# cwozny/sdr_channelizer

Hardware: AMD Instinct MI355X
Metric: input MS/s (complex) channelized (higher is better)
Workload: dtype f32; 1 GPU; cfg2: M=64 channels, 12 taps/branch, D=64, int16 I/Q (12-bit), 2^30 samples per GPU per step, frame-major complex64 out; kernel=pfb_fast<M64,P12,D64,int16>, schedule=default (4: FIR/FFT wave pairs, 8x64-frame workgroups), samples_per_gpu=1073741824, prewarm_steps=20, parallelism=single GPU

## Files before the change

sdr_channelizer_amd/csrc/pfb_fast_core.hpp:

```cpp
#pragma once

#include "pfb_fast_cfg.hpp"

namespace pfb {

template <class K, bool CM = false, bool MS = false>
struct FastKernel : FastRows<K> {
  static constexpr int M = K::M, P = K::P, D = K::D, CPT = K::CPT, C = K::C, W = K::W, OS = K::OS, NT = K::NT;
  static constexpr int NW = W - 1 + C;

  template <int I, bool FULL = false, int MAGSEL = -1, int NTSEL = -1>
  PFB_DEV void pass(const KernelParams& p, float2* src, float2* dst, int tid, long long f0,
                    const v2f (&tw)[2][16]) {
    float2* const p_out = p.out;
    const long long p_frames = p.frames;
    const int nontemporal = NTSEL < 0 ? p.nontemporal : NTSEL;
    constexpr int R = K::R(I), S = K::S(I), KK = K::K(I), RS = K::RS(I);
    constexpr int IPF = M / R, ITEMS = C * IPF, ITERS = (ITEMS + NT - 1) / NT;
    constexpr bool LAST = (I == K::NP - 1);
    constexpr bool TW_REGS = (ITERS == 1) && !K::TW_TABLE;
    constexpr bool READ_BARRIER = !LAST && !K::PINGPONG && NT > 64;
    constexpr bool kMagStaged = MS && LAST;
#pragma unroll
    for (int it = 0; it < ITERS; ++it) {
      const int w = tid + it * NT;
      const bool active = (ITEMS % NT == 0) || (w < ITEMS);
      const int fc = w / IPF, item = w % IPF;
      const int kk = item / S, rest = item % S;
      v2f x[R];
      if (active) {
        const v2f* s2 = reinterpret_cast<const v2f*>(src) + fc * K::FS + item;
#pragma unroll
        for (int n = 0; n < R; ++n) x[n] = s2[n * RS];
      } else {
#pragma unroll
        for (int n = 0; n < R; ++n) x[n] = (v2f){0.f, 0.f};
      }
      if constexpr (READ_BARRIER) __syncthreads();
      Dft<R>::run(x);
      if constexpr (!LAST) {
        constexpr int S1 = K::S(I + 1), RS1 = K::RS(I + 1);
        if constexpr (TW_REGS) {
#pragma unroll
          for (int k = 1; k < R; ++k) x[k] = cmul_w(x[k], tw[I][k]);
        } else {
          const float4* t4 = reinterpret_cast<const float4*>(p.tw_lane + K::TW_OFF(I) + rest * K::TWR(I));
#pragma unroll
          for (int k2 = 0; k2 < K::TWR(I) / 2; ++k2) {
            const float4 t = t4[k2];
            if (k2 > 0) x[2 * k2] = cmul_w(x[2 * k2], (v2f){t.x, t.y});
            if (2 * k2 + 1 < R) x[2 * k2 + 1] = cmul_w(x[2 * k2 + 1], (v2f){t.z, t.w});
          }
        }
        const int n1 = rest / S1, rest2 = rest % S1;
        if (active) {
          v2f* d2 = reinterpret_cast<v2f*>(dst) + fc * K::FS + n1 * RS1 + kk * S1 + rest2;
#pragma unroll
          for (int k = 0; k < R; ++k) d2[k * KK * S1] = x[k];
        }
      } else {
        if constexpr (kMagStaged) {
          static_assert(!CM && NT == 64 && ITERS == 1 && K::NP == 2 && !K::PINGPONG && M % 4 == 0, "single-wave two-pass plans");
          {
            constexpr int SR = M + ((8 - M % 64) + 64) % 64;
            static_assert(C * SR * sizeof(float) <= K::BUF * sizeof(float2), "the staged magnitudes fit the chunk buffer");
            float* stage = reinterpret_cast<float*>(src);
            const int shift = (p.flags & PFB_FLAG_FFTSHIFT) ? (M / 2) : 0;
            team_sync<true>();
#pragma unroll
            for (int k = 0; k < R; ++k) {
              int col = kk + k * KK + shift;
              col = col >= M ? col - M : col;
              if (active) stage[fc * SR + col] = mag_out(x[k].x, x[k].y, p.flags);
            }
            team_sync<true>();
            constexpr int NV = C * M / 4;
#pragma unroll
            for (int j = 0; j < (NV + 63) / 64; ++j) {
              const int idx = tid + 64 * j, fr = idx / (M / 4), q = idx % (M / 4);
              if ((NV % 64 == 0 || idx < NV) && f0 + fr < p_frames) {
                const float4 v = *reinterpret_cast<const float4*>(stage + fr * SR + q * 4);
                *reinterpret_cast<float4*>(reinterpret_cast<float*>(p_out) + (f0 + fr) * M + q * 4) = v;
              }
            }
            return;
          }
        }
        const long long f = f0 + fc;
        if (active && (FULL || f < p_frames)) {
          const bool flip_odd = (OS == 2) && (p.flags & PFB_FLAG_DEROTATE) && ((p.frame0 + f) & 1);
          const v2f sg0 = splat((flip_odd && (kk & 1)) ? -1.f : 1.f), sg1 = splat((flip_odd && ((kk + KK) & 1)) ? -1.f : 1.f);
          auto derot = [&](v2f v, int k) { return OS == 2 ? v * (((k * KK) & 1) ? sg1 : sg0) : v; };
          const int shift = (p.flags & PFB_FLAG_FFTSHIFT) ? (M / 2) : 0;
          auto col_of = [&](int ch) {
            const int c2 = ch + shift;
            return c2 >= M ? c2 - M : c2;
          };
          auto slot = [&](auto* rowp, int k) {
            if constexpr (K::POW2) {
              auto* lo = rowp + kk + shift;
              auto* hi = rowp + kk + (M / 2 - shift);
              return (k < R / 2) ? lo + k * KK : hi + (k - R / 2) * KK;
            } else {
              return rowp + col_of(kk + k * KK);
            }
          };
          if constexpr (CM || (!K::POW2 && K::NT == 64)) {
            const bool mag = MAGSEL < 0 ? (p.flags & PFB_FLAG_MAGNITUDE) != 0 : MAGSEL == 1;
            const long long esz = mag ? 4 : 8;
            const long long cs = CM ? p.out_ld : 1;
            int col = col_of(kk);
            char* ptr = reinterpret_cast<char*>(p_out) + ((long long)col * cs + (CM ? p.out_frame0 + f : f * M)) * esz;
            const long long step = (long long)KK * cs * esz, wrap = (long long)M * cs * esz;
#pragma unroll
            for (int k = 0; k < R; ++k) {
              v2f v = x[k];
              if (mag) {
                *reinterpret_cast<float*>(ptr) = mag_out(v.x, v.y, p.flags);
              } else {
                v = derot(v, k);
                store_c64(reinterpret_cast<float2*>(ptr), v, nontemporal);
              }
              asm volatile("" : "+v"(ptr) : : "memory");
              col += KK;
              ptr += step;
              if (col >= M) { col -= M; ptr -= wrap; }
            }
          } else if (MAGSEL == 1 || (MAGSEL < 0 && (p.flags & PFB_FLAG_MAGNITUDE))) {
            float* rowm = reinterpret_cast<float*>(p_out) + f0 * M + fc * M;
#pragma unroll
            for (int k = 0; k < R; ++k) *slot(rowm, k) = mag_out(x[k].x, x[k].y, p.flags);
          } else {
            float2* row = p_out + f0 * M + fc * M;
#pragma unroll
            for (int k = 0; k < R; ++k) {
              const v2f v = derot(x[k], k);
              store_c64(slot(row, k), v, nontemporal);
            }
          }
        }
      }
    }
  }

  PFB_DEV int tslot_frame(int col, int fc) {
    constexpr int IPF = M / K::R(K::NP - 1), NFC = IPF >= 16 ? 1 : 16 / IPF, Q = 16 / C;
    static_assert(16 % C == 0 && (IPF >= 16 || 16 % IPF == 0) && C % NFC == 0, "power-of-two chunk and lane groups");
    return fc ^ (NFC * ((col / Q) % (C / NFC)));
  }

  PFB_DEV void last_pass_transposed(const KernelParams& p, float2* slot, int tid, long long f0) {
    constexpr int I = K::NP - 1;
    constexpr int R = K::R(I), KK = K::K(I), RS = K::RS(I);
    constexpr int IPF = M / R, ITEMS = C * IPF, ITERS = (ITEMS + NT - 1) / NT;
    static_assert(NT == 64 && !K::PINGPONG && K::S(I) == 1 && M * C <= K::LDS_ELEMS, "wave-local, in place");
    v2f x[ITERS][R];
#pragma unroll
    for (int it = 0; it < ITERS; ++it) {
      const int w = tid + it * NT;
      const bool active = (ITEMS % NT == 0) || (w < ITEMS);
      const int fc = w / IPF, item = w % IPF;
      const v2f* s2 = reinterpret_cast<const v2f*>(slot) + fc * K::FS + item;
#pragma unroll
      for (int n = 0; n < R; ++n) x[it][n] = active ? s2[n * RS] : (v2f){0.f, 0.f};
    }
    team_sync<true>();
    const int shift = (p.flags & PFB_FLAG_FFTSHIFT) ? (M / 2) : 0;
    v2f* t2 = reinterpret_cast<v2f*>(slot);
#pragma unroll
    for (int it = 0; it < ITERS; ++it) {
      const int w = tid + it * NT;
      const bool active = (ITEMS % NT == 0) || (w < ITEMS);
      const int fc = w / IPF, kk = w % IPF;
      Dft<R>::run(x[it]);
      if (active) {
        const bool flip_odd = (OS == 2) && (p.flags & PFB_FLAG_DEROTATE) && ((p.frame0 + f0 + fc) & 1);
        const v2f sg0 = splat((flip_odd && (kk & 1)) ? -1.f : 1.f), sg1 = splat((flip_odd && ((kk + KK) & 1)) ? -1.f : 1.f);
        int col = kk + shift;
        if (col >= M) col -= M;
#pragma unroll
        for (int k = 0; k < R; ++k) {
          v2f v = x[it][k];
          if constexpr (OS == 2) v = v * (((k * KK) & 1) ? sg1 : sg0);
          t2[col * C + tslot_frame(col, fc)] = v;
          col += KK;
          if (col >= M) col -= M;
        }
      }
    }
  }

  struct Consts {
    v2f hp[(W + 1) / 2][CPT];
    v2f tw[2][16];
    int upos[OS][CPT];
    v2f conj_mul;
  };

  PFB_DEV float tap(const Consts& k, int j, int cc) { return (j & 1) ? k.hp[j >> 1][cc].y : k.hp[j >> 1][cc].x; }

  PFB_DEV void setup(const KernelParams& p, int tid, Consts& k) {
    const int c0 = tid * CPT;
#pragma unroll
    for (int cc = 0; cc < CPT; ++cc) {
      const int col = (K::LANES < NT && c0 >= D) ? 0 : c0 + cc;
      const float4* tl = reinterpret_cast<const float4*>(p.taps_lane + (size_t)col * K::WP);
#pragma unroll
      for (int q4 = 0; q4 < K::WP / 4; ++q4) {
        const float4 v = tl[q4];
        if (2 * q4 < (W + 1) / 2) k.hp[2 * q4][cc] = (v2f){v.x, v.y};
        if (2 * q4 + 1 < (W + 1) / 2) k.hp[2 * q4 + 1][cc] = (v2f){v.z, v.w};
      }
    }
    k.conj_mul = (v2f){1.f, (p.flags & PFB_FLAG_CONJUGATE_INPUT) ? -1.f : 1.f};
#pragma unroll
    for (int i = 0; i < K::NP - 1; ++i) {
      constexpr int dummy = 0; (void)dummy;
      const int R = K::R(i), S = K::S(i), IPF = M / R;
      if (C * IPF <= NT && !K::TW_TABLE) {
        const int rest = (tid % IPF) % S;
        const float4* t4 = reinterpret_cast<const float4*>(p.tw_lane + K::TW_OFF(i) + rest * K::TWR(i));
#pragma unroll
        for (int k2 = 0; k2 < 8; ++k2) {
          if (2 * k2 < R) {
            const float4 v = t4[k2];
            k.tw[i][2 * k2] = (v2f){v.x, v.y};
            k.tw[i][2 * k2 + 1] = (v2f){v.z, v.w};
          }
        }
      }
    }
#pragma unroll
    for (int ph = 0; ph < OS; ++ph)
#pragma unroll
      for (int cc = 0; cc < CPT; ++cc) {
        const int n = (D - 1 - (c0 + cc)) + D * ph;
        k.upos[ph][cc] = (n / K::S(0)) * K::RS(0) + (n % K::S(0));
      }
  }

  template <bool WAVE_LOCAL = false, bool TRANSPOSED = false, bool FULL = false, int MAGSEL = -1>
  PFB_DEV void fir_fft_store(const KernelParams& p, const Consts& k, const v2f (&x)[NW][CPT], float2* lds, int tid,
                             long long f0) {
    float2* buf0 = lds;
    float2* buf1 = K::PINGPONG ? lds + K::BUF : lds;
#pragma unroll
    for (int ph = 0; ph < OS; ++ph)
#pragma unroll
      for (int cc = 0; cc < CPT; ++cc) {
        v2f acc[C];
        int tok = 0;
#pragma unroll
        for (int q = 0; q < P; ++q) {
          const int j = ph + OS * q;
#pragma unroll
          for (int t = 0; t < C; ++t) {
            if (q == 0 && (j & 1)) fma_tap0_hi(acc[t], x[W - 1 + t - j][cc], k.hp[j >> 1][cc]);
            else if (q == 0) fma_tap0_lo(acc[t], x[W - 1 + t - j][cc], k.hp[j >> 1][cc]);
            else if (j & 1) fma_tap_hi(acc[t], x[W - 1 + t - j][cc], k.hp[j >> 1][cc], tok);
            else fma_tap_lo(acc[t], x[W - 1 + t - j][cc], k.hp[j >> 1][cc], tok);
          }
        }
        if (!(K::LANES < NT) || tid < K::LANES) {
#pragma unroll
          for (int t = 0; t < C; ++t)
            reinterpret_cast<v2f*>(buf0)[t * K::FS + k.upos[ph][cc]] = acc[t] * k.conj_mul;
        }
      }
    team_sync<WAVE_LOCAL>();
    pass<0>(p, buf0, buf1, tid, f0, k.tw);
    team_sync<WAVE_LOCAL>();
    if constexpr (TRANSPOSED) {
      static_assert(K::NP == 2 && WAVE_LOCAL, "single-wave two-pass plans");
      last_pass_transposed(p, buf1, tid, f0);
      return;
    } else if constexpr (K::NP == 2) {
      pass<1, FULL, MAGSEL>(p, buf1, nullptr, tid, f0, k.tw);
    } else {
      pass<1>(p, buf1, buf0, tid, f0, k.tw);
      team_sync<WAVE_LOCAL>();
      pass<2, FULL, MAGSEL>(p, buf0, nullptr, tid, f0, k.tw);
    }
    team_sync<WAVE_LOCAL>();
  }

  static constexpr bool kPairWrite = CPT == 2 && K::RS(0) == K::S(0) && K::S(0) % 2 == 0 && D % 2 == 0 && K::FS % 2 == 0 &&
                                     K::BUF % 2 == 0;
  PFB_DEV void fir_to_lds(const Consts& k, const v2f (&x)[NW][CPT], float2* buf, int tid) {
    if constexpr (kPairWrite) {
#pragma unroll
      for (int ph = 0; ph < OS; ++ph) {
        v2f acc[2][C];
#pragma unroll
        for (int cc = 0; cc < 2; ++cc) {
          int tok = 0;
#pragma unroll
          for (int q = 0; q < P; ++q) {
            const int j = ph + OS * q;
#pragma unroll
            for (int t = 0; t < C; ++t) {
              if (q == 0 && (j & 1)) fma_tap0_hi(acc[cc][t], x[W - 1 + t - j][cc], k.hp[j >> 1][cc]);
              else if (q == 0) fma_tap0_lo(acc[cc][t], x[W - 1 + t - j][cc], k.hp[j >> 1][cc]);
              else if (j & 1) fma_tap_hi(acc[cc][t], x[W - 1 + t - j][cc], k.hp[j >> 1][cc], tok);
              else fma_tap_lo(acc[cc][t], x[W - 1 + t - j][cc], k.hp[j >> 1][cc], tok);
            }
          }
        }
        if (!(K::LANES < NT) || tid < K::LANES) {
#pragma unroll
          for (int t = 0; t < C; ++t) {
            const v2f lo = acc[1][t] * k.conj_mul, hi = acc[0][t] * k.conj_mul;
            *reinterpret_cast<float4*>(buf + t * K::FS + k.upos[ph][1]) = make_float4(lo.x, lo.y, hi.x, hi.y);
          }
        }
      }
      return;
    }
#pragma unroll
    for (int ph = 0; ph < OS; ++ph)
#pragma unroll
      for (int cc = 0; cc < CPT; ++cc) {
        v2f acc[C];
        int tok = 0;
#pragma unroll
        for (int q = 0; q < P; ++q) {
          const int j = ph + OS * q;
#pragma unroll
          for (int t = 0; t < C; ++t) {
            if (q == 0 && (j & 1)) fma_tap0_hi(acc[t], x[W - 1 + t - j][cc], k.hp[j >> 1][cc]);
            else if (q == 0) fma_tap0_lo(acc[t], x[W - 1 + t - j][cc], k.hp[j >> 1][cc]);
            else if (j & 1) fma_tap_hi(acc[t], x[W - 1 + t - j][cc], k.hp[j >> 1][cc], tok);
            else fma_tap_lo(acc[t], x[W - 1 + t - j][cc], k.hp[j >> 1][cc], tok);
          }
        }
        if (!(K::LANES < NT) || tid < K::LANES) {
#pragma unroll
          for (int t = 0; t < C; ++t)
            reinterpret_cast<v2f*>(buf)[t * K::FS + k.upos[ph][cc]] = acc[t] * k.conj_mul;
        }
      }
  }

  template <bool FULL = false, int MAGSEL = -1, int NTSEL = -1>
  PFB_DEV void fft_from_lds(const KernelParams& p, const Consts& k, float2* buf, int tid, long long f0) {
    static_assert(K::NP == 2 && !K::PINGPONG, "two in-place passes");
    pass<0>(p, buf, buf, tid, f0, k.tw);
    team_sync<true>();
    pass<1, FULL, MAGSEL, NTSEL>(p, buf, nullptr, tid, f0, k.tw);
  }
};

}
```

sdr_channelizer_amd/csrc/pfb_fast_teams.hpp:

```cpp
#pragma once

#include "pfb_fast_core.hpp"

namespace pfb {

template <class K>
struct Teams : FastKernel<K> {
  using F = FastKernel<K>;
  using typename F::raw_t; using typename F::Consts;
  using F::cvt; using F::setup; using F::fir_to_lds;
  static constexpr int M = K::M, P = K::P, D = K::D, CPT = K::CPT, C = K::C, W = K::W, OS = K::OS, NT = K::NT, NW = F::NW;

  template <int I>
  PFB_DEV void pass_frame(const KernelParams& p, float2* fbuf, int lane, const v2f (&tw)[2][16]) {
    constexpr int R = K::R(I), S = K::S(I), KK = K::K(I), RS = K::RS(I);
    constexpr int IPF = M / R, ITERS = (IPF + 63) / 64;
    constexpr int S1 = K::S(I + 1), RS1 = K::RS(I + 1);
    static_assert(I < K::NP - 1, "the last pass (with the stores) belongs to the FIR team");
    constexpr bool TW_REGS = (ITERS == 1) && !K::TW_TABLE;
    v2f x[ITERS][R];
#pragma unroll
    for (int it = 0; it < ITERS; ++it) {
      const int item = lane + it * 64;
      const bool active = (IPF % 64 == 0) || (item < IPF);
      const v2f* s2 = reinterpret_cast<const v2f*>(fbuf) + (active ? item : 0);
#pragma unroll
      for (int n = 0; n < R; ++n) x[it][n] = s2[n * RS];
    }
#pragma unroll
    for (int it = 0; it < ITERS; ++it) {
      const int item = lane + it * 64;
      const bool active = (IPF % 64 == 0) || (item < IPF);
      const int kk = item / S, rest = item % S;
      Dft<R>::run(x[it]);
      if constexpr (TW_REGS) {
#pragma unroll
        for (int k = 1; k < R; ++k) x[it][k] = cmul_w(x[it][k], tw[I][k]);
      } else {
        const float4* t4 = reinterpret_cast<const float4*>(p.tw_lane + K::TW_OFF(I) + (active ? rest : 0) * K::TWR(I));
#pragma unroll
        for (int k2 = 0; k2 < K::TWR(I) / 2; ++k2) {
          const float4 t = t4[k2];
          if (k2 > 0) x[it][2 * k2] = cmul_w(x[it][2 * k2], (v2f){t.x, t.y});
          if (2 * k2 + 1 < R) x[it][2 * k2 + 1] = cmul_w(x[it][2 * k2 + 1], (v2f){t.z, t.w});
        }
      }
      if (active) {
        const int n1 = rest / S1, rest2 = rest % S1;
        v2f* d2 = reinterpret_cast<v2f*>(fbuf) + n1 * RS1 + kk * S1 + rest2;
#pragma unroll
        for (int k = 0; k < R; ++k) d2[k * KK * S1] = x[it][k];
      }
    }
  }

  template <bool INTERIOR, int MAGSEL = -1>
  PFB_DEV void fir_team(const KernelParams& p, const Consts& k, float2* bufs, long long f_begin, int nch) {
    const int tid = threadIdx.x;
    const int c0 = tid * CPT;
    auto last_pass = [&](float2* buf, int c) {
      int t2 = tid;
      asm volatile("" : "+v"(t2));
      F::template pass<K::NP - 1, INTERIOR, MAGSEL>(p, buf, nullptr, t2, f_begin + (long long)c * C, k.tw);
    };
    const raw_t* run_ptr = static_cast<const raw_t*>(p.in) + ((f_begin - (W - 1)) * D + p.base);
    v2f x[NW][CPT];
    raw_t raw[2][C][CPT];
#pragma unroll
    for (int i = 0; i < W - 1; ++i) {
      raw_t t[CPT];
      F::template load_row<INTERIOR>(p, run_ptr, f_begin - (W - 1) + i, i, c0, t);
#pragma unroll
      for (int cc = 0; cc < CPT; ++cc) x[i][cc] = cvt(t[cc]);
    }
#pragma unroll
    for (int u = 0; u < 2; ++u)
#pragma unroll
      for (int t = 0; t < C; ++t) F::template load_row<INTERIOR>(p, run_ptr, f_begin + u * C + t, W - 1 + u * C + t, c0, raw[u][t]);
    int b_fir = 0, b_last = 1;
    auto step = [&]<int U, bool LASTP>(int ci) {
      const long long f0 = f_begin + (long long)ci * C;
#pragma unroll
      for (int t = 0; t < C; ++t)
#pragma unroll
        for (int cc = 0; cc < CPT; ++cc) x[W - 1 + t][cc] = cvt(raw[U][t][cc]);
      if (ci + 2 < nch) {
        const long long rel = (long long)(ci + 2) * C + (W - 1);
#pragma unroll
        for (int t = 0; t < C; ++t) F::template load_row<INTERIOR>(p, run_ptr, f0 + 2 * C + t, rel + t, c0, raw[U][t]);
      }
      fir_to_lds(k, x, bufs + b_fir * K::BUF, tid);
#pragma unroll
      for (int i = 0; i < W - 1; ++i)
#pragma unroll
        for (int cc = 0; cc < CPT; ++cc) x[i][cc] = x[i + C][cc];
      if constexpr (LASTP) last_pass(bufs + b_last * K::BUF, ci - 2);
      __syncthreads();
      b_fir = (b_fir == 2) ? 0 : b_fir + 1;
      b_last = (b_last == 2) ? 0 : b_last + 1;
    };
    step.template operator()<0, false>(0);
    step.template operator()<1, false>(1);
    for (int ci2 = 2; ci2 < nch; ci2 += 2) {
      step.template operator()<0, true>(ci2);
      step.template operator()<1, true>(ci2 + 1);
    }
    if (nch >= 2) last_pass(bufs + b_last * K::BUF, nch - 2);
    __syncthreads();
    b_last = (b_last == 2) ? 0 : b_last + 1;
    last_pass(bufs + b_last * K::BUF, nch - 1);
  }

  template <int MAGSEL = -1>
  PFB_DEV void run_teams(const KernelParams& p, float2* bufs) {
    static_assert(K::NP == 3 && !K::PINGPONG && NT % 64 == 0, "three in-place passes");
    const int wave = threadIdx.x >> 6, lane = threadIdx.x & 63;
    const int nch = p.frames_per_block / C;
    Consts k;
    setup(p, wave < NT / 64 ? threadIdx.x : lane, k);
    long long run = blockIdx.x;
    run = xcd_remap_block(run, gridDim.x, p.xcd_remap);
    const long long f_begin = run * p.frames_per_block;
    if (f_begin >= p.frames) return;
    if (wave < NT / 64) {
      const bool interior = p.vec_ok && ((f_begin - (W - 1)) * D + p.base >= 0) && (f_begin + p.frames_per_block <= p.frames);
      if (interior) fir_team<true, MAGSEL>(p, k, bufs, f_begin, nch);
      else fir_team<false, MAGSEL>(p, k, bufs, f_begin, nch);
    } else {
      const int fr = wave - NT / 64;
      int b = 0;
#pragma unroll 1
      for (int s = 0; s <= nch; ++s) {
        if (s >= 1) {
          float2* fbuf = bufs + b * K::BUF + fr * K::FS;
          pass_frame<0>(p, fbuf, lane, k.tw);
          team_sync<true>();
          pass_frame<1>(p, fbuf, lane, k.tw);
          b = (b == 2) ? 0 : b + 1;
        }
        __syncthreads();
      }
    }
  }
};

template <class K>
constexpr bool kTeamsOk = !K::WAVE_FRAMES && K::NP == 3 && !K::PINGPONG && K::NT > 64 && (K::NT + 64 * K::C) <= 1024 &&
                          3 * sizeof(float2) * K::BUF <= 160 * 1024 && K::C % 2 == 0;

template <class K, bool MAG>
__global__ void __launch_bounds__(K::NT + 64 * K::C, K::MIN_WAVES) pfb_teams_kernel(const KernelParams p) {
  carry_history(p, SampleT<K::FMT>::kBytes, K::NT + 64 * K::C);
  __shared__ float2 bufs[3 * K::BUF];
  Teams<K>::template run_teams<MAG ? 1 : 0>(p, bufs);
}

template <class K>
KernelEntry teams_entry(const KernelParams& p) {
  static constexpr KernelTag mag = kernel_tag<>("teams", {.magsel = 1}), c64 = kernel_tag<>("teams", {.magsel = 0});
  return wants_magnitude(p) ? entry_for(&pfb_teams_kernel<K, true>, 6, mag.s, p, p.frames_per_block, K::NT + 64 * K::C)
                            : entry_for(&pfb_teams_kernel<K, false>, 6, c64.s, p, p.frames_per_block, K::NT + 64 * K::C);
}

}
```

Baseline: 484,800 MS/s.

## Peel interior FIR loop, use scalar-base prefetch loads, clamp last-pass lanes

The interior FIR team loop is restructured. The steady-state iterations now prefetch unconditionally, and the final two steps are peeled so they skip the prefetch. Prefetch loads use a new scalar-base-plus-vector-offset global load so address math stays in SGPRs, and sched_barriers plus an explicit waitcnt constrain instruction scheduling. The last FFT pass clamps out-of-range work items to a duplicate valid item instead of branching on activity. These changes aim to cut per-step address and branch overhead, but depend on hand-placed waitcnt encodings and scheduling fences that may reduce compiler freedom.

```diff
diff --git a/sdr_channelizer_amd/csrc/pfb_fast_core.hpp b/sdr_channelizer_amd/csrc/pfb_fast_core.hpp
--- a/sdr_channelizer_amd/csrc/pfb_fast_core.hpp
+++ b/sdr_channelizer_amd/csrc/pfb_fast_core.hpp
@@ -9,7 +9,7 @@
   static constexpr int M = K::M, P = K::P, D = K::D, CPT = K::CPT, C = K::C, W = K::W, OS = K::OS, NT = K::NT;
   static constexpr int NW = W - 1 + C;
 
-  template <int I, bool FULL = false, int MAGSEL = -1, int NTSEL = -1>
+  template <int I, bool FULL = false, int MAGSEL = -1, int NTSEL = -1, bool DUP = false>
   PFB_DEV void pass(const KernelParams& p, float2* src, float2* dst, int tid, long long f0,
                     const v2f (&tw)[2][16]) {
     float2* const p_out = p.out;
@@ -23,7 +23,7 @@
     constexpr bool kMagStaged = MS && LAST;
 #pragma unroll
     for (int it = 0; it < ITERS; ++it) {
-      const int w = tid + it * NT;
+      const int w = (DUP && tid + it * NT >= ITEMS) ? ITEMS - 1 : tid + it * NT;
       const bool active = (ITEMS % NT == 0) || (w < ITEMS);
       const int fc = w / IPF, item = w % IPF;
       const int kk = item / S, rest = item % S;
diff --git a/sdr_channelizer_amd/csrc/pfb_fast_teams.hpp b/sdr_channelizer_amd/csrc/pfb_fast_teams.hpp
--- a/sdr_channelizer_amd/csrc/pfb_fast_teams.hpp
+++ b/sdr_channelizer_amd/csrc/pfb_fast_teams.hpp
@@ -54,14 +54,28 @@
     }
   }
 
+  PFB_DEV void load_row_sbase(const raw_t* rowp, unsigned cbyte, raw_t (&raw)[CPT]) {
+    using RawVec = typename F::RawVec;
+    static_assert(sizeof(RawVec) % 4 == 0, "whole dwords per lane");
+    typedef unsigned dwords_t __attribute__((ext_vector_type(sizeof(RawVec) / 4)));
+    typedef const char __attribute__((address_space(1))) * gbytes_t;
+    uintptr_t base = reinterpret_cast<uintptr_t>(rowp);
+    asm volatile("" : "+s"(base), "+v"(cbyte));
+    const dwords_t v = *reinterpret_cast<const dwords_t __attribute__((address_space(1)))*>(
+        reinterpret_cast<gbytes_t>(base) + cbyte);
+    __builtin_memcpy(&raw[0], &v, sizeof(RawVec));
+  }
+
   template <bool INTERIOR, int MAGSEL = -1>
   PFB_DEV void fir_team(const KernelParams& p, const Consts& k, float2* bufs, long long f_begin, int nch) {
     const int tid = threadIdx.x;
     const int c0 = tid * CPT;
+    unsigned cbyte = ((K::LANES < NT && c0 >= D) ? 0 : c0) * (unsigned)sizeof(raw_t);
+    asm volatile("" : "+v"(cbyte));
     auto last_pass = [&](float2* buf, int c) {
       int t2 = tid;
       asm volatile("" : "+v"(t2));
-      F::template pass<K::NP - 1, INTERIOR, MAGSEL>(p, buf, nullptr, t2, f_begin + (long long)c * C, k.tw);
+      F::template pass<K::NP - 1, INTERIOR, MAGSEL, -1, INTERIOR>(p, buf, nullptr, t2, f_begin + (long long)c * C, k.tw);
     };
     const raw_t* run_ptr = static_cast<const raw_t*>(p.in) + ((f_begin - (W - 1)) * D + p.base);
     v2f x[NW][CPT];
@@ -77,14 +91,24 @@
     for (int u = 0; u < 2; ++u)
 #pragma unroll
       for (int t = 0; t < C; ++t) F::template load_row<INTERIOR>(p, run_ptr, f_begin + u * C + t, W - 1 + u * C + t, c0, raw[u][t]);
+    constexpr int kNone = 0, kAlways = 1, kClamped = 2;
     int b_fir = 0, b_last = 1;
-    auto step = [&]<int U, bool LASTP>(int ci) {
+    auto step = [&]<int U, bool LASTP, int PREF>(int ci) {
       const long long f0 = f_begin + (long long)ci * C;
 #pragma unroll
       for (int t = 0; t < C; ++t)
 #pragma unroll
-        for (int cc = 0; cc < CPT; ++cc) x[W - 1 + t][cc] = cvt(raw[U][t][cc]);
-      if (ci + 2 < nch) {
+        for (int cc = 0; cc < CPT; ++cc) {
+          x[W - 1 + t][cc] = cvt(raw[U][t][cc]);
+          if constexpr (K::FMT == PFB_FMT_CF32) asm("v_mov_b64 %0, %1" : "=v"(x[W - 1 + t][cc]) : "v"(x[W - 1 + t][cc]));
+        }
+      __builtin_amdgcn_sched_barrier(0);
+      if constexpr (INTERIOR && PREF != kNone) {
+        const int cn = (PREF == kClamped && ci + 2 >= nch) ? nch - 1 : ci + 2;
+        const raw_t* rows = run_ptr + ((long long)cn * C + (W - 1)) * D;
+#pragma unroll
+        for (int t = 0; t < C; ++t) load_row_sbase(rows + t * D, cbyte, raw[U][t]);
+      } else if (PREF == kAlways || (PREF == kClamped && ci + 2 < nch)) {
         const long long rel = (long long)(ci + 2) * C + (W - 1);
 #pragma unroll
         for (int t = 0; t < C; ++t) F::template load_row<INTERIOR>(p, run_ptr, f0 + 2 * C + t, rel + t, c0, raw[U][t]);
@@ -96,14 +120,26 @@
         for (int cc = 0; cc < CPT; ++cc) x[i][cc] = x[i + C][cc];
       if constexpr (LASTP) last_pass(bufs + b_last * K::BUF, ci - 2);
       __syncthreads();
+      __builtin_amdgcn_sched_barrier(0);
       b_fir = (b_fir == 2) ? 0 : b_fir + 1;
       b_last = (b_last == 2) ? 0 : b_last + 1;
     };
-    step.template operator()<0, false>(0);
-    step.template operator()<1, false>(1);
-    for (int ci2 = 2; ci2 < nch; ci2 += 2) {
-      step.template operator()<0, true>(ci2);
-      step.template operator()<1, true>(ci2 + 1);
+    step.template operator()<0, false, kClamped>(0);
+    step.template operator()<1, false, kClamped>(1);
+    if constexpr (!INTERIOR) {
+      for (int ci2 = 2; ci2 < nch; ci2 += 2) {
+        step.template operator()<0, true, kClamped>(ci2);
+        step.template operator()<1, true, kClamped>(ci2 + 1);
+      }
+    } else if (nch > 2) {
+      __builtin_amdgcn_s_waitcnt(0x0f70);
+#pragma unroll 1
+      for (int ci2 = 2; ci2 + 2 < nch; ci2 += 2) {
+        step.template operator()<0, true, kAlways>(ci2);
+        step.template operator()<1, true, kAlways>(ci2 + 1);
+      }
+      step.template operator()<0, true, kNone>(nch - 2);
+      step.template operator()<1, true, kNone>(nch - 1);
     }
     if (nch >= 2) last_pass(bufs + b_last * K::BUF, nch - 2);
     __syncthreads();
```

Result: no change. 485,000 MS/s (median of 2 runs) (+0.0%).
